# eBay/KPRN

Measured on AMD Instinct MI355X. Metric: paths/sec (train+score) at path_len=6 d=64, higher is better.
Workload: dtype f32

## Files before the change

### kprn_amd/csrc/kprn_api.hip

```cpp
#include <ctype.h>
#include <dlfcn.h>
#include <errno.h>
#include <math.h>
#include <stdio.h>
#include <string.h>

#include <algorithm>
#include <thread>

#include "kprn_internal.h"

static thread_local std::string g_create_error;

ProfScope::ProfScope(kprn_handle* h_, const char* n, hipStream_t on) : h(h_), name(n), strm(on ? on : h_->stream) {
  if (!h->prof_on) return;
  if (!h->prof_filter.empty() && strncmp(n, h->prof_filter.c_str(), h->prof_filter.size()) != 0) return;
  auto get = [&]() {
    hipEvent_t e;
    if (!h->event_pool.empty()) { e = h->event_pool.back(); h->event_pool.pop_back(); }
    else if (hipEventCreate(&e) != hipSuccess) e = nullptr;
    return e;
  };
  a = get(); b = get();
  if (a) hipEventRecord(a, strm);
// ... 1760 lines not shown
    HIP_TRY(hipEventSynchronize(e1));
    float t = 0.f;
    HIP_TRY(hipEventElapsedTime(&t, e0, e1));
    *ms = t / (float)iters;
  } catch (...) { dfree(A); dfree(B); dfree(C); dfree(X); dfree(Z); hipEventDestroy(e0); hipEventDestroy(e1); throw; }
  dfree(A); dfree(B); dfree(C); dfree(X); dfree(Z); hipEventDestroy(e0); hipEventDestroy(e1);
  API_END(h)
}

int kprn_set_option(kprn_handle* h, const char* key, const char* value) {
  API_BEGIN(h)
  KPRN_REQUIRE(key && value, KPRN_E_ARG, "NULL argument");
  if (strcmp(key, "impl") == 0) {
    if (strcmp(value, "auto") == 0) h->impl = 0;
    else if (strcmp(value, "generic") == 0) h->impl = 1;
    else throw KprnError{KPRN_E_ARG, "impl must be auto or generic"};
  } else if (strcmp(key, "prefix_plan") == 0) {
    h->prefix_plan = atoi(value) ? 1 : 0;
  } else if (strcmp(key, "small_tiles") == 0) {
    join_score(h);
    h->small_tiles_on = atoi(value) != 0;
  } else if (strcmp(key, "tile_handover") == 0) {
    const int v = atoi(value);
    KPRN_REQUIRE(v >= 0 && v <= 2, KPRN_E_ARG, "tile_handover must be 0, 1 or 2");
    h->tile_handover = v;
  } else if (strcmp(key, "rank_sort_min") == 0) {
    const int v = atoi(value);
    KPRN_REQUIRE(v >= 257 && v <= 4097, KPRN_E_ARG, "rank_sort_min must be in 257..4097");
    h->rank_sort_min = v;
  } else if (strcmp(key, "adam_merged") == 0) {
    h->adam_merged = atoi(value) != 0;
  } else if (strcmp(key, "bwd_pipe") == 0) {
    h->bwd_pipe = atoi(value) != 0;
  } else if (strcmp(key, "score_dual") == 0) {
    const int v = atoi(value);
    KPRN_REQUIRE(v >= 0 && v <= 2, KPRN_E_ARG, "score_dual must be 0, 1 or 2");
    h->score_dual = v;
  } else if (strcmp(key, "catchup_prefix") == 0) {
    h->catchup_prefix = atoi(value) != 0;
  } else if (strcmp(key, "fused_small_tables") == 0) {
    h->fused_small_tables = atoi(value) != 0;
  } else if (strcmp(key, "persist_layers") == 0) {
    const int v = atoi(value);
    KPRN_REQUIRE(v >= 0 && v <= 2, KPRN_E_ARG, "persist_layers must be 0, 1 or 2");
    h->persist_layers = v;
  } else if (strcmp(key, "small_tables") == 0) {
    h->small_tables = atoi(value) != 0;
  } else if (strcmp(key, "small_tables_fwd") == 0) {
    join_score(h);
    h->small_tables_fwd = atoi(value) != 0;
  } else if (strcmp(key, "head_select") == 0) {
    join_score(h);
    h->head_select = atoi(value) != 0;
  } else if (strcmp(key, "bf16_t_pad") == 0) {
    bf16p::set_t_pad(atoi(value));
  } else if (strcmp(key, "bf16_gemm_regstage") == 0) {
    bf16p::set_gemm_regstage(atoi(value) != 0);
  } else if (strcmp(key, "bf16_gemm_touch") == 0) {
    bf16p::set_gemm_touch(atoi(value));
  } else if (strcmp(key, "bf16_gemm_pingpong") == 0) {
    bf16p::set_gemm_pingpong(atoi(value) != 0);
  } else if (strcmp(key, "bf16_bptt_dxe") == 0) {
    const int v = atoi(value);
    KPRN_REQUIRE(v == 0 || v == 8 || v == 16, KPRN_E_ARG, "bf16_bptt_dxe must be 0, 8 or 16");
    h->bf16_bptt_dxe = v;
  } else if (strcmp(key, "bf16_small_tables") == 0) {
    h->bf16_small_tables = atoi(value) != 0;
  } else if (strcmp(key, "score_rest_before_bptt") == 0) {
    join_score(h);
    h->score_rest_before_bptt = atoi(value) ? 1 : 0;
  } else if (strcmp(key, "score_rest_in_backward") == 0) {
    join_score(h);
    h->score_rest_in_backward = atoi(value) ? 1 : 0;
    h->after_bptt_hook = h->score_rest_in_backward ? score_rest_hook : nullptr;
  } else if (strcmp(key, "score_split") == 0) {
    join_score(h);
    const double f = atof(value);
    KPRN_REQUIRE(f >= 0.0 && f < 1.0, KPRN_E_ARG, "score_split: a fraction in [0, 1)");
    h->score_split = (float)f;
  } else if (strcmp(key, "score_overlap") == 0) {
    join_score(h);
    h->score_overlap = atoi(value) ? 1 : 0;
  } else if (strcmp(key, "loss_accumulate") == 0) {
    h->loss_accumulate = atoi(value) ? 1 : 0;
  } else if (strcmp(key, "inline_upload") == 0) {
    if (strcmp(value, "side") == 0) h->inline_upload_side = 1;
    else if (strcmp(value, "main") == 0) h->inline_upload_side = 0;
    else throw KprnError{KPRN_E_ARG, "inline_upload must be side or main"};
  } else if (strcmp(key, "train_step_return") == 0) {
    if (strcmp(value, "loss") == 0) h->train_step_drain = 0;
    else if (strcmp(value, "drain") == 0) h->train_step_drain = 1;
    else throw KprnError{KPRN_E_ARG, "train_step_return must be loss or drain"};
  } else if (strcmp(key, "feed_build") == 0) {
    if (strcmp(value, "host") == 0) h->feed_build_host = 1;
    else if (strcmp(value, "device") == 0) h->feed_build_host = 0;
    else throw KprnError{KPRN_E_ARG, "feed_build must be host or device"};
  } else if (strcmp(key, "feed_threads") == 0) {
    const int v = atoi(value);
    KPRN_REQUIRE(v >= 1 && v <= 64, KPRN_E_ARG, "feed_threads must be in 1..64");
    h->feed_threads = v;
  } else if (strcmp(key, "feed_workers") == 0) {
    const int v = atoi(value);
    KPRN_REQUIRE(v >= 1 && v <= 64 && !h->feed_pool, KPRN_E_ARG, "feed_workers must be in 1..64 and set before the first feed");
    h->feed_workers = v;
  } else if (strcmp(key, "profile_filter") == 0) {
    h->prof_filter = value;
// ... 40 lines not shown
```

### kprn_amd/csrc/kprn_internal.h

```cpp
#pragma once
#include <stdlib.h>
#include <hip/hip_runtime.h>
#include <stdint.h>
#include <exception>
#include <functional>
#include <future>
#include <string>
#include <vector>
#include <map>

#include "../../include/kprn.h"
#include "philox_dev.h"

#define KPRN_MAX_LAYERS 8

struct KprnError { int code; std::string msg; };
#define HIP_TRY(expr)                                                                     \
  do {                                                                                    \
    hipError_t e__ = (expr);                                                              \
    if (e__ != hipSuccess)                                                                \
      throw KprnError{KPRN_E_DEVICE, std::string(#expr) + ": " + hipGetErrorString(e__)}; \
  } while (0)
#define KPRN_REQUIRE(cond, code, text) \
  do { if (!(cond)) throw KprnError{(code), std::string(text)}; } while (0)
// ... 123 lines not shown
  const int32_t* rows_view = nullptr; const int32_t* count_view = nullptr; const kprn_batch* view_batch = nullptr;
  bool pad_clean = false;
  bool dense_grads_clean = false;
  int64_t caught_serial = -1, caught_step = -1;
  int64_t grads_serial = -1;
  int64_t next_serial = 1;
  int loss_accumulate = 0;
  float* loss_partial = nullptr; int64_t loss_partial_cap = 0; int loss_pending = 0;
  float* loss_mirror = nullptr; int64_t loss_mirror_cap = 0; hipEvent_t ev_loss = nullptr;
  bool loss_early_armed = false; int loss_early_n = 0; int train_step_drain = 0;
  float* probs_mirror = nullptr; int64_t probs_mirror_cap = 0; float* sel_host_armed = nullptr;
  int32_t* dp_mark = nullptr;
  bool dp_fused_update = false, dp_union_pending = false;
  const void* dp_all = nullptr; int dp_world = 0, dp_cap = 0;
  void* dp_comm = nullptr; int dp_rank = 0, dp_nranks = 0;
  int32_t* dp_gather = nullptr; int64_t dp_gather_words = 0;
  bool dp_comm_stream_on = false, dp_begun = false;
  hipStream_t dp_comm_stream = nullptr; hipEvent_t ev_dp_packed = nullptr, ev_dp_gathered = nullptr;
  bool dp_dense_in_pack = false;
  bool dp_saved_dense_in_pack = false, dp_saved_fused_update = false;
  int32_t* pack_buf = nullptr; int64_t pack_cap = 0, pack_words = 0;

  float* d_loss = nullptr;
  float* d_norm2 = nullptr;
  int32_t* d_flag = nullptr;
  float* h_pinned = nullptr;

  Workspace ws;
  float* score_buf = nullptr;
  void* fused_state = nullptr;
  void* bf16_state = nullptr;
  void* bidx_scratch = nullptr; size_t bidx_scratch_bytes = 0;
  hipStream_t feed_stream = nullptr; hipEvent_t ev_feed_fork = nullptr;
  void* feed_scratch = nullptr; size_t feed_scratch_bytes = 0;
  int feed_build_host = 1;
  int feed_workers = 0, feed_threads = 0;
  void* feed_pool = nullptr;
  void* upload_pool = nullptr;
  hipStream_t upload_stream = nullptr;
  int impl = 0;
  int prefix_plan = 1;
  int score_overlap = 0;
  hipStream_t score_stream = nullptr;
  int side_stream_probes = 0;
  hipEvent_t ev_fork = nullptr, ev_score_done = nullptr;
  kprn_batch* dropin_slot[4] = {nullptr, nullptr, nullptr, nullptr};
  int dropin_next_train = 0, dropin_next_score = 0, dropin_last = 0;
  bool dropin_prev_waited = false, dropin_prev_waited_now = false; int inline_upload_side = 1;
  bool inline_side_ok = true;
  bool score_pending = false;
  int bf16_bptt_dxe = 8;
  int persist_layers = 1;
  bool small_tables_fwd = true;
  bool head_select = true;
  bool small_tables = true;
  float* lp_wot = nullptr; int64_t lp_wot_cap = 0;
  float* st_ctmp = nullptr; int64_t st_ctmp_cap = 0;
  bool bf16_small_tables = true;
  bool small_tiles_on = true;
  int tile_handover = 2; int* ho_fault = nullptr;
  bool adam_merged = true;
  bool bwd_pipe = true;
  int score_dual = 2;
  bool catchup_prefix = true;
  bool fused_small_tables = true;
  float score_split = 0.f;
  int score_rest_in_backward = 0;
  int score_rest_before_bptt = 0;
  hipStream_t rest_stream = nullptr; hipEvent_t ev_part1 = nullptr;
  void (*after_bptt_hook)(kprn_handle*) = nullptr;
  const kprn_batch* score_rest_batch = nullptr; int score_rest_cid = 1; int64_t score_rest_tile0 = 0;
  bool last_forward_side = false;
  bool score_on_main = false;
  const kprn_batch* pool_defer_batch = nullptr; int pool_defer_cid = 0;
  float* S2 = nullptr; float* sel2 = nullptr; int64_t cap_N2 = 0, cap_B2 = 0;
  int reserve_cus = 0;
  int32_t last_B = 0;
  float* board = nullptr; int64_t board_n = 0;
  hipEvent_t ev_put = nullptr; bool put_side = false;
  void* rank_buf = nullptr; size_t rank_buf_bytes = 0;
  int rank_sort_min = 512;
  void* rank_pin = nullptr; size_t rank_pin_bytes = 0, rank_pin_off[2] = {0, 0};
  void* explain_buf = nullptr; size_t explain_buf_bytes = 0;
  void* explain_pin = nullptr; size_t explain_pin_bytes = 0;
  std::vector<kprn_graph*> graphs;
  void* pf_buf = nullptr; size_t pf_buf_bytes = 0;
  std::vector<kprn_sampler*> samplers;
  void* ns_buf = nullptr; size_t ns_buf_bytes = 0;

  int deterministic = 0;
  DetScratch det_slab;
  float* det_seg = nullptr; int64_t det_seg_cap = 0;
  float dropout_p = 0.f;
  uint64_t dropout_seed = 0;
  uint32_t drop_draw = 0, drop_draw_cur = 0;
  bool drop_live = false;
  float* det_norm_part = nullptr;

  bool prof_on = false;

  std::string prof_filter;
  std::map<std::string, ProfEntry> prof;
  struct Pending { std::string name; hipEvent_t a, b;  int launches = 1; };
  std::vector<Pending> prof_pending;
  std::vector<hipEvent_t> event_pool;
};
// ... 429 lines not shown
```

### kprn_amd/csrc/lstm_fused_bwd.hip

```cpp
#include <string.h>

#include <memory>

#include "lstm_fused_common.h"

namespace fused {

struct BwdArgs {
  const int32_t* idx; int64_t N; int T, F, nT;
  const float *Wt, *We, *Wr; int dt, de, dr; int Vt, Vr;
  int L, layer;
  const float* WiT;
  const float* WoT;
  const float* save_frag;
  const float* dS;
  const float* wout_row;
  float* gWout_row; float* gbout_c;
  float* DX;
  float* DXe;
  int64_t Npad;
  float* gWi; float* gbi; float* gWo;
  float* gWt; float* gWe; float* gWr;
  float* part;
  unsigned long long* timing;
  int dbg;
  int64_t n_tiles;
  const int32_t* tile_k;
  float* PG;
  HoArgs ho;
  int small_lds;
  float* gG;
  unsigned* pipe_flag;
  int pipe;
};


constexpr int PART = 2 * 256 * 64 + 256;
constexpr int NS_ID = 16;
constexpr int PART_G = PART + 256 * NS_ID;
constexpr int LDD = 4 * DH + 4;
constexpr int DET_PG = 80, DET_SMALL = DET_PG + (KCAP + 1) * PFB, DET_STRIDE = DET_SMALL + 1024;

#ifdef KPRN_TIMING_PROBES
#define KPRN_PROBES_ON 1
#else
#define KPRN_PROBES_ON 0
#endif
#define TPROBE(slot)                                                                 \
  if (KPRN_PROBES_ON && a.timing) {                                                   \
    const unsigned long long now__ = __builtin_amdgcn_s_memtime();                    \
    tacc[slot] += now__ - tlast;                                                      \
    tlast = now__;                                                                    \
  }

struct Pre {
  f32x4 P[6];
  f32x4 up;
  f32x4 bin[4];
  f32x4 bhp[4];
};

__device__ __forceinline__ void gather_load_ident(const BwdArgs& a, const int t, const int32_t* ids, f32x4 (&v)[4]) {
  const int ch = threadIdx.x & 15, c0 = 4 * ch;
  const int32_t* p = ids + t * MT + (threadIdx.x >> 4);
  const float* eb = a.We - a.de + ((ch + 4) & 7) * 4;
#pragma unroll
  for (int k = 0; k < 4; ++k) {
    const f32x4 e = *(const f32x4*)(eb + (int64_t)p[IDS_PLANE<MT> + k * 16] * a.de);
    const int rel = p[2 * IDS_PLANE<MT> + k * 16] - 1, typ = a.Vr + p[k * 16] - 1;
    f32x4 oh;
#pragma unroll
    for (int i = 0; i < 4; ++i) oh[i] = (c0 + i == rel || c0 + i == typ) ? 1.f : 0.f;
    v[k] = (ch < 4) ? oh : ((ch < 12) ? e : f32x4{0.f, 0.f, 0.f, 0.f});
  }
}

template <bool BOTTOM, bool TOP, int NMT, bool IDENT = false, bool DET = false>
__device__ __forceinline__ void bwd_body(const BwdArgs& a, const int bx, const int G_, float* const det_part = nullptr) {
  static_assert(!IDENT || (BOTTOM && !TOP && NMT == 4), "the identity route: bottom layer of two, 64-path tiles");
  constexpr int MTR = 16 * NMT;
  constexpr int NXT = IDENT ? 3 : 4;
  extern __shared__ __attribute__((aligned(16))) float lds[];
  unsigned long long tacc[8] = {0, 0, 0, 0, 0, 0, 0, 0};
  unsigned long long tlast = (KPRN_PROBES_ON && a.timing) ? __builtin_amdgcn_s_memtime() : 0ull;
  float* dA_t = lds;
  float* in_t = dA_t + MT * LDD;
  int32_t* ids = (int32_t*)(in_t + (BOTTOM ? MT * LDA : 0));
  constexpr int IDS_BUF = MT * MAXT_LDS * 4;
  float* pg = (float*)(ids + (BOTTOM ? 2 * IDS_BUF : 0));

  const int tid = threadIdx.x;
  const int lane = tid & 63;
  const int j = __builtin_amdgcn_readfirstlane(tid >> 6);
  const int arow = lane & 15, ag = lane >> 4;
  const int T = a.T, L = a.L, ly = a.layer;
  const HoPlan ho = ho_plan(a.ho, a.tile_k, a.n_tiles, T, 1, bx, G_);
  auto mof = [&](const int i) -> int { return IDENT ? ((i + 2 * (j >> 1)) & 3) : i; };
  if (IDENT && bx == 0) for (int c = tid; c < 256 * NS_ID; c += 256) a.gG[c] = 0.f;

  f32x4 wiT[16], woT[16];
  {
    const float* wi_row = a.WiT + (int64_t)((IDENT ? a.dt + 16 * (j & 1) : j * 16) + arow) * (4 * DH) + ag * 4;
    const float* wo_row = a.WoT + (int64_t)(j * 16 + arow) * (4 * DH) + ag * 4;
#pragma unroll
    for (int S = 0; S < 16; ++S) { wiT[S] = *(const f32x4*)(wi_row + S * 16); woT[S] = *(const f32x4*)(wo_row + S * 16); }
#pragma unroll
    for (int S = 0; S < 16; ++S) { asm volatile("" : "+a"(wiT[S])); asm volatile("" : "+a"(woT[S])); }
  }
  f32x4 dwi[4][4], dwo[4][4];
  float dbias[4];
#pragma unroll
  for (int q = 0; q < 4; ++q) {
    dbias[q] = 0.f;
#pragma unroll
    for (int nt = 0; nt < 4; ++nt) {
      dwi[q][nt] = f32x4{0.f, 0.f, 0.f, 0.f}; dwo[q][nt] = f32x4{0.f, 0.f, 0.f, 0.f};
      if (nt < NXT) asm volatile("" : "+a"(dwi[q][nt]));
      asm volatile("" : "+a"(dwo[q][nt]));
    }
  }

  const int64_t frag_unit = (int64_t)NPL * 256;
  const int64_t frag_mt_stride = (int64_t)T * L * 4 * frag_unit;
  const int wcls = (j * 16 < a.dt) ? 0 : ((j * 16 < a.dt + a.de) ? 1 : 2);
  GatherSrc gsrc;
  if (BOTTOM) gsrc = gather_src(a);
  const float wout_c = TOP ? a.wout_row[j * 16 + arow] : 0.f;
  float gwo = 0.f, gbo = 0.f;
  for (int c = tid; c < (KCAP + 1) * PFB; c += 256) pg[c] = 0.f;
  f32x4 sacc[2] = {f32x4{0.f, 0.f, 0.f, 0.f}, f32x4{0.f, 0.f, 0.f, 0.f}};
  TPROBE(0)

  const int64_t n_mine = (a.n_tiles > (int64_t)bx) ? (a.n_tiles - 1 - bx) / G_ + 1 : 0;
  float* const ho_slot = a.ho.state + (int64_t)ho.slot * HO_STATE + threadIdx.x * 4;
  auto own_of = [&](const int64_t it) -> int64_t {
    const int64_t ti = TOP ? n_mine - 1 - it : ((ho.role == 1) ? (it + 1 < n_mine ? it + 1 : 0) : it);
    return (int64_t)bx + ti * G_;
  };
  int ipar = 1;
  int k0_req = 0;
  auto request_tile = [&](const int64_t tl, const int buf) {
    if (a.tile_k) k0_req = a.tile_k[tl];
    if (BOTTOM) ids_stage_dma<256, MTR>(a.idx, a.N, T, a.F, a.nT, tl, ids + buf * IDS_BUF);
  };
  if (n_mine > 0) request_tile(ho.role == 2 ? ho.tile : own_of(0), 0);
  for (int64_t it = 0; it < n_mine; ++it) {
    const int64_t own_tile = own_of(it);
    const bool late = ho.role == 1 && own_tile == (int64_t)bx;
    const bool early = ho.role == 2 && it == 0;
    int64_t tile, n0;
    int k0, Te;
    const float* frag_tile;
    float* dx_tile;
    auto retarget = [&](const int64_t tl) {
      tile = tl;
      n0 = tl * MTR;
      k0 = a.tile_k ? __builtin_amdgcn_readfirstlane(k0_req) : 0;
      Te = T - k0;
      frag_tile = a.save_frag + tl * NMT * frag_mt_stride + (int64_t)k0 * L * 4 * frag_unit + lane * 4;
      dx_tile = a.DX + (((tl * NMT) * T + k0) * 4 + j) * 256 + lane * 4;
    };
    retarget(early ? ho.tile : own_tile);
    auto frag_ptr = [&](int mt, int t, int l, int w, int plane) -> const float* {
      return frag_tile + mt * frag_mt_stride + ((int64_t)(t * L + l) * 4 + w) * frag_unit + plane * 256;
    };
    f32x4 P[6], up, bin[4], bhp[4];
    auto load_P = [&](const int slot, int t) {
      const int mt = mof(slot);
#pragma unroll
      for (int k = 0; k < 6; ++k) P[k] = *(const f32x4*)frag_ptr(mt, t, ly, j, k);
      if constexpr (!TOP && NMT == 1) {
        if (a.pipe == 2) {
          const unsigned* fl = a.pipe_flag + tile * MAXT_LDS + (k0 + t);
          const long long t0 = wall_clock64();
          while (__hip_atomic_load(fl, __ATOMIC_RELAXED, __HIP_MEMORY_SCOPE_AGENT) != a.ho.epoch) {
            __builtin_amdgcn_s_sleep(4);
            if (wall_clock64() - t0 > HO_TIMEOUT_TICKS) {
              if (threadIdx.x == 0) __hip_atomic_store(a.ho.fault, 1, __ATOMIC_RELAXED, __HIP_MEMORY_SCOPE_SYSTEM);
              break;
            }
          }
          asm volatile("" ::: "memory");
          up = ho_load4(dx_tile + (mt * T + t) * 1024);
        } else up = *(const f32x4*)(dx_tile + (mt * T + t) * 1024);
      } else if (!TOP) up = *(const f32x4*)(dx_tile + (mt * T + t) * 1024);
    };
    auto load_B = [&](int nt, const int slot, int t, bool has_hp) {
      const int mt = mof(slot);
      if (!BOTTOM) bin[nt] = *(const f32x4*)frag_ptr(mt, t, ly - 1, nt, 6);
      if (has_hp) bhp[nt] = *(const f32x4*)frag_ptr(mt, t - 1, ly, nt, 6);
    };
    auto load_bin_lds = [&](int nt, const int slot) {
      if (nt >= NXT) return;
      const int mt = mof(slot);
#pragma unroll
      for (int r = 0; r < 4; ++r) bin[nt][r] = in_t[(mt * 16 + ag * 4 + r) * LDA + nt * 16 + arow];
    };
    auto gather_load_x = [&](const int t, f32x4 (&v)[MTR * 16 / 256]) {
      if constexpr (IDENT) gather_load_ident(a, t, ids + ipar * IDS_BUF, v);
      else gather_load_planes<256, MTR>(a, gsrc, tile, t, ids + ipar * IDS_BUF, v);
    };
    const int tt_hi = late ? Te - 1 - ho.d : Te - 1;
    f32x4 dc[NMT], dh[NMT];
    auto init_state = [&]() {
#pragma unroll
      for (int m = 0; m < NMT; ++m) {
        dc[m] = f32x4{0.f, 0.f, 0.f, 0.f};
        dh[m] = f32x4{0.f, 0.f, 0.f, 0.f};
        if (TOP) {
          const f32x4 hf = *(const f32x4*)(frag_tile + m * frag_mt_stride + ((int64_t)((Te - 1) * L + ly) * 4 + j) * frag_unit + 6 * 256);
#pragma unroll
          for (int r = 0; r < 4; ++r) {
            const int64_t n = n0 + m * 16 + ag * 4 + r;
            const float d = (n < a.N) ? a.dS[n] : 0.f;
            dh[m][r] = d * wout_c;
            gwo += d * hf[r];
            gbo += d;
          }
        }
      }
    };
    if (__builtin_expect(late, 0)) {
      ho_wait(a.ho, ho.slot);
#pragma unroll
      for (int m = 0; m < NMT; ++m) { dh[m] = ho_load4(ho_slot + m * 1024); dc[m] = ho_load4(ho_slot + (NMT + m) * 1024); }
    } else {
      init_state();
    }
    auto tile_prologue = [&](const int tt_first, const int64_t next) {
      ipar ^= 1;
      if (BOTTOM) {
        asm volatile("s_waitcnt vmcnt(0)" ::: "memory");
        lds_barrier();
        f32x4 nin[MTR * 16 / 256];
        gather_load_x(k0 + tt_first, nin);
        gather_store<256, MTR>(in_t, nin);
      }
      if (next >= 0) request_tile(next, ipar ^ 1);
      if (BOTTOM) lds_barrier();
    };
    tile_prologue(tt_hi, early ? own_tile : (it + 1 < n_mine ? own_of(it + 1) : (int64_t)-1));
    TPROBE(1)
    load_P(0, tt_hi);
#pragma unroll
    for (int nt = 0; nt < 4; ++nt) load_B(nt, 0, tt_hi, tt_hi > 0);

    auto step = [&](auto rec_tag, const int t) {
      constexpr bool REC = decltype(rec_tag)::value;
      if (BOTTOM) {
#pragma unroll
        for (int nt = 0; nt < 4; ++nt) load_bin_lds(nt, 0);
      }
#pragma unroll
      for (int mt = 0; mt < NMT; ++mt) {
        f32x4 dhv = dh[mt];
        if (!TOP) dhv += up;
        const f32x4 dC = dc[mt] + dhv * P[4];
        f32x4 dA[4];
        dA[0] = dC * P[0];
        dA[1] = dC * P[1];
        dA[2] = dC * P[2];
        dA[3] = dhv * P[3];
        dc[mt] = dC * P[5];
#pragma unroll
        for (int q = 0; q < 4; ++q) {
#pragma unroll
          for (int r = 0; r < 4; ++r) dA_t[(mof(mt) * 16 + ag * 4 + r) * LDD + q * DH + j * 16 + arow] = dA[q][r];
          dbias[q] += (dA[q][0] + dA[q][1]) + (dA[q][2] + dA[q][3]);
        }
        __builtin_amdgcn_sched_barrier(0);
        TPROBE(7)
        if (mt < NMT - 1) load_P(mt + 1, t);
        else if (REC) load_P(0, t - 1);
#pragma unroll
        for (int nt = 0; nt < 4; ++nt) {
#pragma unroll
          for (int r = 0; r < 4; ++r)
#pragma unroll
            for (int q = 0; q < 4; ++q) {
              if (nt < NXT) KPRN_MFMA_ACC_A(dwi[q][nt], dA[q][r], bin[nt][r]);
              if (REC) KPRN_MFMA_ACC_A(dwo[q][nt], dA[q][r], bhp[nt][r]);
            }
          __builtin_amdgcn_sched_barrier(0);
          if (mt < NMT - 1) { load_B(nt, mt + 1, t, REC); if (BOTTOM) load_bin_lds(nt, mt + 1); }
          else if (REC) load_B(nt, 0, t - 1, t > 1);
        }
        TPROBE(2)
      }
      lds_barrier();
      if (!REC && k0 > 0) {
        float cs0 = 0.f, cs1 = 0.f;
#pragma unroll 8
        for (int row = 0; row < MTR; row += 2) { cs0 += dA_t[row * LDD + tid]; cs1 += dA_t[(row + 1) * LDD + tid]; }
        pg[k0 * PFB + tid] += cs0 + cs1;
      }
      TPROBE(3)
      f32x4 nin[MTR * 16 / 256];
      if (BOTTOM && REC) gather_load_x(k0 + t - 1, nin);

      f32x4 ax[4], ah[4];
      if constexpr (NMT < 4) {
#pragma unroll
        for (int q = NMT; q < 4; ++q) { ax[q] = f32x4{0.f, 0.f, 0.f, 0.f}; ah[q] = f32x4{0.f, 0.f, 0.f, 0.f}; }
      }
      if constexpr (IDENT) { ax[2] = f32x4{0.f, 0.f, 0.f, 0.f}; ax[3] = f32x4{0.f, 0.f, 0.f, 0.f}; }
      if constexpr (IDENT) {
        const float* abase = dA_t + arow * LDD + ag * 4;
        auto afrag = [&](const int slot, const int S) { return *(const f32x4*)(abase + mof(slot) * 16 * LDD + S * 16); };
        if (REC) {
          f32x4 p0 = afrag(0, 0), p1, p2, p3;
#pragma unroll
          for (int S = 0; S < 16; ++S) {
#pragma unroll
            for (int i = 0; i < 2; ++i) {
              const f32x4 a4 = (i == 0) ? p0 : p1;
              if (S == 0) { KPRN_MFMA_Z(ax[i], a4[0], wiT[S][0]); KPRN_MFMA_Z(ah[i], a4[0], woT[S][0]); }
              else { KPRN_MFMA(ax[i], a4[0], wiT[S][0]); KPRN_MFMA(ah[i], a4[0], woT[S][0]); }
              KPRN_MFMA(ax[i], a4[1], wiT[S][1]); KPRN_MFMA(ah[i], a4[1], woT[S][1]);
              if (i == 0) p1 = afrag(1, S);
              else { p2 = afrag(2, S); p3 = afrag(3, S); }
              KPRN_MFMA(ax[i], a4[2], wiT[S][2]); KPRN_MFMA(ah[i], a4[2], woT[S][2]);
              KPRN_MFMA(ax[i], a4[3], wiT[S][3]); KPRN_MFMA(ah[i], a4[3], woT[S][3]);
            }
            const f32x4 a2 = p2, a3 = p3;
            if (S == 0) { KPRN_MFMA_Z(ah[2], a2[0], woT[S][0]); KPRN_MFMA_Z(ah[3], a3[0], woT[S][0]); }
            else { KPRN_MFMA(ah[2], a2[0], woT[S][0]); KPRN_MFMA(ah[3], a3[0], woT[S][0]); }
            KPRN_MFMA(ah[2], a2[1], woT[S][1]); KPRN_MFMA(ah[3], a3[1], woT[S][1]);
            if (S + 1 < 16) p0 = afrag(0, S + 1);
            KPRN_MFMA(ah[2], a2[2], woT[S][2]); KPRN_MFMA(ah[3], a3[2], woT[S][2]);
            KPRN_MFMA(ah[2], a2[3], woT[S][3]); KPRN_MFMA(ah[3], a3[3], woT[S][3]);
          }
        } else {
          f32x4 p0 = afrag(0, 0), p1 = afrag(1, 0);
#pragma unroll
          for (int S = 0; S < 16; ++S) {
            const f32x4 a0 = p0, a1 = p1;
            if (S == 0) { KPRN_MFMA_Z(ax[0], a0[0], wiT[S][0]); KPRN_MFMA_Z(ax[1], a1[0], wiT[S][0]); }
            else { KPRN_MFMA(ax[0], a0[0], wiT[S][0]); KPRN_MFMA(ax[1], a1[0], wiT[S][0]); }
// ... 6 lines not shown
      } else {
        const float* abase = dA_t + arow * LDD + ag * 4;
        if (REC) {
          f32x4 apre = *(const f32x4*)(abase);
#pragma unroll
          for (int S = 0; S < 16; ++S) {
#pragma unroll
            for (int mt = 0; mt < NMT; ++mt) {
              const f32x4 a4 = apre;
              const int gn = S * NMT + mt + 1;
              if (S == 0) { KPRN_MFMA_Z(ax[mt], a4[0], wiT[S][0]); KPRN_MFMA_Z(ah[mt], a4[0], woT[S][0]); }
              else { KPRN_MFMA(ax[mt], a4[0], wiT[S][0]); KPRN_MFMA(ah[mt], a4[0], woT[S][0]); }
              KPRN_MFMA(ax[mt], a4[1], wiT[S][1]); KPRN_MFMA(ah[mt], a4[1], woT[S][1]);
              if (gn < 16 * NMT) apre = *(const f32x4*)(abase + (gn % NMT) * 16 * LDD + (gn / NMT) * 16);
              KPRN_MFMA(ax[mt], a4[2], wiT[S][2]); KPRN_MFMA(ah[mt], a4[2], woT[S][2]);
              KPRN_MFMA(ax[mt], a4[3], wiT[S][3]); KPRN_MFMA(ah[mt], a4[3], woT[S][3]);
            }
          }
        } else if constexpr (NMT == 1) {
          f32x4 ap0 = *(const f32x4*)(abase), ap1 = *(const f32x4*)(abase + 16);
#pragma unroll
          for (int S = 0; S < 16; S += 2) {
            const f32x4 a0 = ap0, a1 = ap1;
            if (S == 0) { KPRN_MFMA_Z(ax[0], a0[0], wiT[S][0]); KPRN_MFMA_Z(ax[1], a1[0], wiT[S + 1][0]); }
            else { KPRN_MFMA(ax[0], a0[0], wiT[S][0]); KPRN_MFMA(ax[1], a1[0], wiT[S + 1][0]); }
            KPRN_MFMA(ax[0], a0[1], wiT[S][1]); KPRN_MFMA(ax[1], a1[1], wiT[S + 1][1]);
            if (S + 2 < 16) { ap0 = *(const f32x4*)(abase + (S + 2) * 16); ap1 = *(const f32x4*)(abase + (S + 3) * 16); }
            KPRN_MFMA(ax[0], a0[2], wiT[S][2]); KPRN_MFMA(ax[1], a1[2], wiT[S + 1][2]);
            KPRN_MFMA(ax[0], a0[3], wiT[S][3]); KPRN_MFMA(ax[1], a1[3], wiT[S + 1][3]);
          }
        } else {
          f32x4 ap0 = *(const f32x4*)(abase), ap1 = *(const f32x4*)(abase + 16 * LDD);
#pragma unroll
          for (int S = 0; S < 16; ++S) {
#pragma unroll
            for (int mp = 0; mp < 2; ++mp) {
              const f32x4 a0 = ap0, a1 = ap1;
              const int gn = S * 2 + mp + 1;
              if (S == 0) { KPRN_MFMA_Z(ax[2 * mp], a0[0], wiT[S][0]); KPRN_MFMA_Z(ax[2 * mp + 1], a1[0], wiT[S][0]); }
              else { KPRN_MFMA(ax[2 * mp], a0[0], wiT[S][0]); KPRN_MFMA(ax[2 * mp + 1], a1[0], wiT[S][0]); }
              KPRN_MFMA(ax[2 * mp], a0[1], wiT[S][1]); KPRN_MFMA(ax[2 * mp + 1], a1[1], wiT[S][1]);
              if (gn < 32) {
                ap0 = *(const f32x4*)(abase + ((gn & 1) * 2) * 16 * LDD + (gn >> 1) * 16);
                ap1 = *(const f32x4*)(abase + ((gn & 1) * 2 + 1) * 16 * LDD + (gn >> 1) * 16);
              }
              KPRN_MFMA(ax[2 * mp], a0[2], wiT[S][2]); KPRN_MFMA(ax[2 * mp + 1], a1[2], wiT[S][2]);
              KPRN_MFMA(ax[2 * mp], a0[3], wiT[S][3]); KPRN_MFMA(ax[2 * mp + 1], a1[3], wiT[S][3]);
            }
          }
        }
      }
      KPRN_MFMA_DRAIN();
      KPRN_PIN_V4(ax);
      if (REC) KPRN_PIN_V4(ah);
      if constexpr (NMT == 1) { if (!REC) ax[0] += ax[1]; }
      if (BOTTOM && REC) gather_store<256, MTR>(in_t, nin);
      const bool compact = !IDENT && BOTTOM && a.DXe != nullptr && wcls == 1;
#pragma unroll
      for (int mt = 0; mt < NMT; ++mt) {
        if (REC) dh[mt] = ah[mt];
        if constexpr (IDENT) continue;
        if constexpr (TOP && !BOTTOM && NMT == 1) {
          if (a.pipe == 1) ho_store4(dx_tile + (mt * T + t) * 1024, ax[mt]);
          else *(f32x4*)(dx_tile + (mt * T + t) * 1024) = ax[mt];
        } else
        if (!compact && !(BOTTOM && a.small_lds && wcls != 1)) *(f32x4*)(dx_tile + (mt * T + t) * 1024) = ax[mt];
      }
      if (compact) {
        float* de_row = a.DXe + ((n0 + ag * 4) * T + k0 + t) * (int64_t)a.de + (j * 16 + arow - a.dt);
#pragma unroll
        for (int mt = 0; mt < NMT; ++mt)
#pragma unroll
          for (int r = 0; r < 4; ++r) de_row[(int64_t)(mt * 16 + r) * T * a.de] = ax[mt][r];
      }
      if constexpr (IDENT) {
        float* de_row = a.DXe + ((n0 + ag * 4) * T + k0 + t) * (int64_t)a.de + 16 * (j & 1) + arow;
#pragma unroll
        for (int i = 0; i < 2; ++i)
#pragma unroll
          for (int r = 0; r < 4; ++r) de_row[(int64_t)(mof(i) * 16 + r) * T * a.de] = ax[i][r];
      }
      if (!IDENT && BOTTOM && a.small_lds && wcls != 1) {
        const int32_t* idp = ids + ipar * IDS_BUF + ((wcls == 0) ? 0 : 2) * IDS_PLANE<MTR> + (k0 + t) * MTR + ag * 4;
#pragma unroll
        for (int mt = 0; mt < NMT; ++mt) {
          const int4 id4 = *(const int4*)(idp + mt * 16);
          const float o0 = (id4.x - 1 == arow) ? 1.f : 0.f, o1 = (id4.y - 1 == arow) ? 1.f : 0.f;
          const float o2 = (id4.z - 1 == arow) ? 1.f : 0.f, o3 = (id4.w - 1 == arow) ? 1.f : 0.f;
          KPRN_MFMA_VV(sacc[0], o0, ax[mt][0]);
          KPRN_MFMA_VV(sacc[1], o1, ax[mt][1]);
          KPRN_MFMA_VV(sacc[0], o2, ax[mt][2]);
          KPRN_MFMA_VV(sacc[1], o3, ax[mt][3]);
        }
        KPRN_MFMA_DRAIN();
        asm volatile("" : "+v"(sacc[0]), "+v"(sacc[1]));
      }
      TPROBE(4)
      if constexpr (TOP && !BOTTOM && NMT == 1) {
        if (a.pipe == 1) asm volatile("s_waitcnt vmcnt(0)" ::: "memory");
      }
      lds_barrier();
      if constexpr (TOP && !BOTTOM && NMT == 1) {
        if (a.pipe == 1 && tid == 0) __hip_atomic_store(a.pipe_flag + tile * MAXT_LDS + (k0 + t), a.ho.epoch, __ATOMIC_RELAXED, __HIP_MEMORY_SCOPE_AGENT);
      }
      TPROBE(5)
    };
    int tt_sw = early ? Te - ho.d : -1;
    int tt_pub = -1;
    for (int tt = tt_hi; tt > 0; --tt) {
      step(std::true_type{}, tt);
      if (__builtin_expect(tt == tt_pub, 0)) { ho_publish(a.ho, ho.slot); tt_pub = -1; }
      if (__builtin_expect(tt == tt_sw, 0)) {
#pragma unroll
        for (int m = 0; m < NMT; ++m) { ho_store4(ho_slot + m * 1024, dh[m]); ho_store4(ho_slot + (NMT + m) * 1024, dc[m]); }
        retarget(own_tile);
        init_state();
        tile_prologue(Te - 1, n_mine > 1 ? own_of(1) : (int64_t)-1);
        load_P(0, Te - 1);
#pragma unroll
        for (int nt = 0; nt < 4; ++nt) load_B(nt, 0, Te - 1, Te > 1);
        tt = Te;
        tt_sw = -1;
        tt_pub = Te - 1;
      }
    }
    step(std::false_type{}, 0);
    if (k0 > 0) {
      float cs = 0.f;
#pragma unroll
      for (int m = 0; m < NMT; ++m) cs += (dc[m][0] + dc[m][1]) + (dc[m][2] + dc[m][3]);
      cs += __shfl_xor(cs, 16, 64);
      cs += __shfl_xor(cs, 32, 64);
      if (ag == 0) pg[k0 * PFB + 4 * DH + j * 16 + arow] += cs;
    }
  }
  float* const det_slab = DET ? det_part + (int64_t)bx * DET_STRIDE : nullptr;
  if (a.tile_k) {
    lds_barrier();
    for (int c = PFB + tid; c < (KCAP + 1) * PFB; c += 256) {
      const float v = pg[c];
      if constexpr (DET) det_slab[DET_PG + c] = v;
      else if (v != 0.f) unsafeAtomicAdd(a.PG + c, v);
    }
  }
  if (!IDENT && BOTTOM && a.small_lds && wcls != 1) {
    const f32x4 sg = sacc[0] + sacc[1];
    const int V = (wcls == 0) ? a.Vt : a.Vr, width = (wcls == 0) ? a.dt : a.dr;
    float* g = (DET ? det_slab + DET_SMALL + ((wcls == 0) ? 0 : a.Vt * a.dt) : ((wcls == 0) ? a.gWt : a.gWr)) + (j * 16 + arow - ((wcls == 0) ? 0 : a.dt + a.de));
#pragma unroll
    for (int i = 0; i < 4; ++i) {
      const int v = 4 * ag + i;
      if constexpr (DET) { if (v < V) g[(int64_t)v * width] = sg[i]; }
      else if (v < V && sg[i] != 0.f) unsafeAtomicAdd(g + (int64_t)v * width, sg[i]);
    }
  }

  KPRN_MFMA_DRAIN();
#pragma unroll
  for (int q = 0; q < 4; ++q) {
    if constexpr (IDENT) asm volatile("" : "+a"(dwi[q][0]), "+a"(dwi[q][1]), "+a"(dwi[q][2]), "+a"(dwo[q][0]), "+a"(dwo[q][1]), "+a"(dwo[q][2]), "+a"(dwo[q][3]));
    else KPRN_PIN_A8(dwi[q], dwo[q]);
  }
  {
    float* pw = a.part + (int64_t)bx * PART_G;
#pragma unroll
    for (int q = 0; q < 4; ++q) {
#pragma unroll
      for (int nt = 0; nt < 4; ++nt) {
#pragma unroll
        for (int r = 0; r < 4; ++r) {
          const int64_t grow = (int64_t)q * DH + j * 16 + ag * 4 + r;
          if constexpr (IDENT) {
            if (nt == 0) pw[PART + grow * NS_ID + arow] = dwi[q][0][r];
            else if (nt < NXT) pw[grow * DH + a.dt + (nt - 1) * 16 + arow] = dwi[q][nt][r];
            else {
              pw[grow * DH + (arow < a.dt ? arow : arow + a.de)] = 0.f;
              pw[grow * DH + (16 + arow < a.dt ? 16 + arow : 16 + arow + a.de)] = 0.f;
            }
          } else {
            pw[grow * DH + nt * 16 + arow] = dwi[q][nt][r];
          }
          pw[256 * 64 + grow * DH + nt * 16 + arow] = dwo[q][nt][r];
        }
      }
      float v = dbias[q];
      v += __shfl_xor(v, 16, 64);
      v += __shfl_xor(v, 32, 64);
      if (ag == 0) pw[2 * 256 * 64 + q * DH + j * 16 + arow] = v;
    }
  }
  if (TOP) {
    float v = gwo;
    v += __shfl_xor(v, 16, 64);
    v += __shfl_xor(v, 32, 64);
    if constexpr (DET) { if (ag == 0) det_slab[j * 16 + arow] = v; }
    else if (ag == 0) unsafeAtomicAdd(a.gWout_row + j * 16 + arow, v);
    float bsum = gbo;
    bsum += __shfl_xor(bsum, 16, 64);
    bsum += __shfl_xor(bsum, 32, 64);
    if constexpr (DET) { if (j == 0 && lane == 0) det_slab[DH] = bsum; }
    else if (j == 0 && lane == 0) unsafeAtomicAdd(a.gbout_c, bsum);
  }
  TPROBE(6)
  if (KPRN_PROBES_ON && a.timing && tid == 0) {
    for (int k = 0; k < 8; ++k) a.timing[(int64_t)bx * 8 + k] = tacc[k];
  }
}

template <bool BOTTOM, bool TOP, int NMT>
__global__ __launch_bounds__(256, 1) void k_lstm_bwd(BwdArgs a) { bwd_body<BOTTOM, TOP, NMT>(a, (int)blockIdx.x, (int)gridDim.x); }
__global__ __launch_bounds__(256, 1) void k_lstm_bwd_ident(BwdArgs a) { bwd_body<true, false, 4, true>(a, (int)blockIdx.x, (int)gridDim.x); }

template <int NMT>
__global__ __launch_bounds__(256, 1) void k_lstm_bwd_dual(BwdArgs top, BwdArgs bottom, int g) {
  if ((int)blockIdx.x < g) bwd_body<false, true, NMT>(top, (int)blockIdx.x, g);
  else bwd_body<true, false, NMT>(bottom, (int)blockIdx.x - g, g);
}

template <bool BOTTOM, bool TOP, int NMT, bool IDENT>
__global__ __launch_bounds__(256, 1) void k_lstm_bwd_det(BwdArgs a, float* det_part) {
  bwd_body<BOTTOM, TOP, NMT, IDENT, true>(a, (int)blockIdx.x, (int)gridDim.x, det_part);
}
template <int NMT>
__global__ __launch_bounds__(256, 1) void k_lstm_bwd_dual_det(BwdArgs top, BwdArgs bottom, int g, float* det_top, float* det_bottom) {
  if ((int)blockIdx.x < g) bwd_body<false, true, NMT, false, true>(top, (int)blockIdx.x, g, det_top);
  else bwd_body<true, false, NMT, false, true>(bottom, (int)blockIdx.x - g, g, det_bottom);
}
struct DetJoin { int nseg, nslab; float* dst[6]; const float* src[6]; int n[6]; int blk0[7]; };
__global__ __launch_bounds__(256) void k_det_join(DetJoin a) {
  constexpr int DEPTH = 16;
  int sgm = 0;
  while (sgm + 1 < a.nseg && (int)blockIdx.x >= a.blk0[sgm + 1]) ++sgm;
  const int i = ((int)blockIdx.x - a.blk0[sgm]) * 256 + threadIdx.x;
  if (i >= a.n[sgm]) return;
  const float* __restrict__ src = a.src[sgm] + i;
  float acc = 0.f;
  for (int w0 = 0; w0 < a.nslab; w0 += DEPTH) {
    float x[DEPTH];
#pragma unroll
    for (int u = 0; u < DEPTH; ++u) x[u] = src[(int64_t)(w0 + u < a.nslab ? w0 + u : a.nslab - 1) * DET_STRIDE];
#pragma unroll
    for (int u = 0; u < DEPTH; ++u) if (w0 + u < a.nslab) acc += x[u];
  }
  a.dst[sgm][i] += acc;
}

struct ScatArgs {
  const int32_t* idx; int64_t N; int T, F, nT;
  int dt, de, dr, Vt, Vr;
  const float* DX;
  float *gWt, *gWe, *gWr;
  const int32_t* tile_k;
  int do_small, do_entity;
  float* part_small;
  int64_t n_tiles;
};

__global__ __launch_bounds__(256) void k_embed_scatter_frag(ScatArgs a) {
  extern __shared__ __attribute__((aligned(16))) float lds[];
  float* dxt = lds;
  int32_t* ids = (int32_t*)(dxt + MT * LDA);
  float* small_g = (float*)(ids + MT * 4);
  const int tid = threadIdx.x, lane = tid & 63, w0 = tid >> 6;
  const int arow = lane & 15, ag = lane >> 4;
  const int T = a.T, D = a.dt + a.de + a.dr;
  const int n_small = a.Vt * a.dt + a.Vr * a.dr;
  const bool small_in_lds = a.part_small != nullptr && a.do_small;
  if (small_in_lds) for (int i = tid; i < n_small; i += 256) small_g[i] = 0.f;
  const int e0 = a.dt, e1 = a.dt + a.de;
  const int col = tid & 63, rg = tid >> 6;
  const int64_t n_items = a.n_tiles * T;
  for (int64_t item = blockIdx.x; item < n_items; item += gridDim.x) {
    const int64_t tile = item / T;
    const int t = (int)(item - tile * T);
// ... 70 lines not shown
    __syncthreads();
    for (int i = tid; i < n_small; i += 256) a.part_small[(int64_t)blockIdx.x * n_small + i] = small_g[i];
  }
}

__global__ __launch_bounds__(256) void k_reduce_small(const float* __restrict__ part, int nslab, int n_small, int nt_small, float* __restrict__ gWt, float* __restrict__ gWr) {
  __shared__ float red[16][17];
  const int e = threadIdx.x & 15, sl = threadIdx.x >> 4;
  const int i = blockIdx.x * 16 + e;
  float acc = 0.f;
  if (i < n_small) for (int s = sl; s < nslab; s += 16) acc += part[(int64_t)s * n_small + i];
  red[sl][e] = acc;
  __syncthreads();
  if (sl == 0 && i < n_small) {
    float v = 0.f;
#pragma unroll
    for (int k = 0; k < 16; ++k) v += red[k][e];
    if (i < nt_small) unsafeAtomicAdd(gWt + i, v); else unsafeAtomicAdd(gWr + (i - nt_small), v);
  }
}

__global__ void k_reduce_partials(bidx::SlabReduce a) { bidx::slab_reduce_block(a, blockIdx.x, blockIdx.y, blockIdx.z); }

struct TransArgs { const float* W[4]; float* WT[4]; };
__global__ void k_transpose_256x64(TransArgs a) {
  const int i = blockIdx.x * blockDim.x + threadIdx.x;
  if (i >= 64 * 256) return;
  const int n = i >> 8, k = i & 255;
  a.WT[blockIdx.y][i] = a.W[blockIdx.y][k * 64 + n];
}

bool transpose_job(kprn_handle* h, kk::TransposeJob* tj) {
  State* s = st(h);
  if (!s->wt_dirty) return false;
  const int L = h->cfg.L;
  if (!s->WT) HIP_TRY(kprn_dev_malloc((void**)&s->WT, (size_t)2 * 2 * 64 * 256 * sizeof(float)));
  tj->n = 2 * L;
  for (int m = 0; m < 4; ++m) {
    const int l = (m >> 1) < L ? (m >> 1) : 0;
    tj->W[m] = h->dense + ((m & 1) ? h->layer[l].Wo : h->layer[l].Wi);
    tj->WT[m] = s->WT + (size_t)(l * 2 + (m & 1)) * 64 * 256;
  }
  s->wt_dirty = false;
  return true;
}

bool bwd_supported(const kprn_handle* h, int T) { return fwd_supported(h, T); }

template <bool BOTTOM, bool TOP, int NMT = 4, bool IDENT = false>
static void launch_bwd(kprn_handle* h, const BwdArgs& a, int grid, float* det_part = nullptr) {
  size_t lds_bytes = (size_t)MT * LDD * sizeof(float);
  if (BOTTOM) lds_bytes += (size_t)MT * LDA * sizeof(float) + 2 * (MT * MAXT_LDS * 4) * sizeof(int32_t);
  lds_bytes += (size_t)(KCAP + 1) * PFB * sizeof(float);
  if (det_part) {
    if constexpr (BOTTOM || TOP) {
      static PerDeviceOnce det_attr_done;
      if (det_attr_done.need())
        HIP_TRY(hipFuncSetAttribute((const void*)k_lstm_bwd_det<BOTTOM, TOP, NMT, IDENT>, hipFuncAttributeMaxDynamicSharedMemorySize, (int)lds_bytes));
      hipLaunchKernelGGL((k_lstm_bwd_det<BOTTOM, TOP, NMT, IDENT>), dim3(grid), dim3(256), lds_bytes, h->stream, a, det_part);
      HIP_TRY(hipGetLastError());
      return;
    }
    throw KprnError{KPRN_E_UNSUPPORTED, "deterministic: the fused path has no middle layer"};
  }
  static PerDeviceOnce attr_done;
  const void* fn = IDENT ? (const void*)k_lstm_bwd_ident : (const void*)k_lstm_bwd<BOTTOM, TOP, NMT>;
  if (attr_done.need()) HIP_TRY(hipFuncSetAttribute(fn, hipFuncAttributeMaxDynamicSharedMemorySize, (int)lds_bytes));
  if constexpr (IDENT) hipLaunchKernelGGL(k_lstm_bwd_ident, dim3(grid), dim3(256), lds_bytes, h->stream, a);
  else hipLaunchKernelGGL((k_lstm_bwd<BOTTOM, TOP, NMT>), dim3(grid), dim3(256), lds_bytes, h->stream, a);
  HIP_TRY(hipGetLastError());
}

void backward(kprn_handle* h, const kprn_batch* b, int cid) {
  const kprn_config& c = h->cfg;
  State* s = st(h);
  const int64_t N = b->N;
  const int T = b->T, L = c.L;
  hipStream_t strm = h->stream;
  if (N > s->cap_Nb || T > s->cap_Tb) {
    HIP_TRY(hipStreamSynchronize(strm));
    if (s->DX) hipFree(s->DX);
    const int64_t cn = std::max<int64_t>(N, s->cap_Nb);
    const int ct = std::max(T, s->cap_Tb);
    HIP_TRY(kprn_dev_malloc((void**)&s->DX, (size_t)ct * (cn + 2 * MT) * DH * sizeof(float)));
    if (s->DXe) hipFree(s->DXe);
    HIP_TRY(kprn_dev_malloc((void**)&s->DXe, (size_t)(ct * (cn + 2 * MT) + KCAP) * c.de * sizeof(float)));
    s->cap_Nb = cn; s->cap_Tb = ct;
  }
  if (!s->part) HIP_TRY(kprn_dev_malloc((void**)&s->part, (size_t)2 * s->num_cu * PART_G * sizeof(float)));
  const bool det = h->deterministic;
  if (det && !s->det_part) HIP_TRY(kprn_dev_malloc((void**)&s->det_part, (size_t)2 * s->num_cu * DET_STRIDE * sizeof(float)));
  static const bool want_timing = KPRN_DEV_ENV("KPRN_TIMING") != nullptr;
  if (want_timing && !s->timing) HIP_TRY(kprn_dev_malloc((void**)&s->timing, (size_t)s->num_cu * 12 * sizeof(unsigned long long)));
  if (s->wt_dirty) {
    ProfScope ps(h, "weight_transpose");
    kk::TransposeJob tj;
    transpose_job(h, &tj);
    TransArgs ta;
    for (int m = 0; m < 4; ++m) { ta.W[m] = tj.W[m < tj.n ? m : 0]; ta.WT[m] = tj.WT[m < tj.n ? m : 0]; }
    hipLaunchKernelGGL(k_transpose_256x64, dim3(64, tj.n), dim3(256), 0, strm, ta);
    HIP_TRY(hipGetLastError());
  }
  float* gd = h->g_dense;
  const bool small = small_tiles(h, N, b->tile_k != nullptr);
  const int64_t n_tiles64 = (N + MT - 1) / MT;
  const int64_t n_tiles = small ? (N + 15) / 16 : n_tiles64;
// ... 207 lines not shown
```

Measured before the change: 51.25 million.

## Stage backward h fragments through LDS with async global-to-LDS loads

Adds a default-on path for the fused LSTM backward kernel (64-path tiles, top or bottom layer of two). It prefetches the previous-step hidden and lower-layer input fragments into a double-buffered LDS area using global_load_lds_dwordx4, so the register loads of B operands inside the MFMA loop become LDS reads. The aim is to hide global-load latency on the recurrent critical path and free VGPRs. In exchange it uses extra LDS, adds vmcnt waits and barriers, and relies on inline asm that manipulates m0.

Measured after the change: 51.27 million, median of 5. No clear change (+0.0%).

```diff
diff --git a/kprn_amd/csrc/kprn_api.hip b/kprn_amd/csrc/kprn_api.hip
--- a/kprn_amd/csrc/kprn_api.hip
+++ b/kprn_amd/csrc/kprn_api.hip
@@ -1836,6 +1836,8 @@
   } else if (strcmp(key, "head_select") == 0) {
     join_score(h);
     h->head_select = atoi(value) != 0;
+  } else if (strcmp(key, "bwd_h_lds") == 0) {
+    h->bwd_h_lds = atoi(value) != 0;
   } else if (strcmp(key, "bf16_t_pad") == 0) {
     bf16p::set_t_pad(atoi(value));
   } else if (strcmp(key, "bf16_gemm_regstage") == 0) {
diff --git a/kprn_amd/csrc/kprn_internal.h b/kprn_amd/csrc/kprn_internal.h
--- a/kprn_amd/csrc/kprn_internal.h
+++ b/kprn_amd/csrc/kprn_internal.h
@@ -199,6 +199,7 @@
   int bf16_bptt_dxe = 8;
   int persist_layers = 1;
   bool small_tables_fwd = true;
+  bool bwd_h_lds = true;
   bool head_select = true;
   bool small_tables = true;
   float* lp_wot = nullptr; int64_t lp_wot_cap = 0;
diff --git a/kprn_amd/csrc/lstm_fused_bwd.hip b/kprn_amd/csrc/lstm_fused_bwd.hip
--- a/kprn_amd/csrc/lstm_fused_bwd.hip
+++ b/kprn_amd/csrc/lstm_fused_bwd.hip
@@ -75,9 +75,12 @@
   }
 }
 
-template <bool BOTTOM, bool TOP, int NMT, bool IDENT = false, bool DET = false>
+template <bool TOP> constexpr int HB_FLOATS = 4 * (TOP ? 2 : 1) * 4 * 256;
+template <bool BOTTOM, bool TOP, int NMT, bool IDENT = false, bool DET = false, bool HLDS = false>
 __device__ __forceinline__ void bwd_body(const BwdArgs& a, const int bx, const int G_, float* const det_part = nullptr) {
   static_assert(!IDENT || (BOTTOM && !TOP && NMT == 4), "the identity route: bottom layer of two, 64-path tiles");
+  static_assert(!HLDS || (NMT == 4 && BOTTOM != TOP), "h fragments through LDS: 64-path tiles, top or bottom layer of two");
+  constexpr int HB_SRC = TOP ? 2 : 1, HB = HB_FLOATS<TOP>;
   constexpr int MTR = 16 * NMT;
   constexpr int NXT = IDENT ? 3 : 4;
   extern __shared__ __attribute__((aligned(16))) float lds[];
@@ -88,6 +91,7 @@
   int32_t* ids = (int32_t*)(in_t + (BOTTOM ? MT * LDA : 0));
   constexpr int IDS_BUF = MT * MAXT_LDS * 4;
   float* pg = (float*)(ids + (BOTTOM ? 2 * IDS_BUF : 0));
+  float* hb = pg + (KCAP + 1) * PFB;
 
   const int tid = threadIdx.x;
   const int lane = tid & 63;
@@ -185,10 +189,32 @@
         } else up = *(const f32x4*)(dx_tile + (mt * T + t) * 1024);
       } else if (!TOP) up = *(const f32x4*)(dx_tile + (mt * T + t) * 1024);
     };
-    auto load_B = [&](int nt, const int slot, int t, bool has_hp) {
+    auto load_B = [&](int nt, const int slot, int t, bool has_hp, const bool tile_start = false) {
+#ifdef KPRN_EXP_BOWN
+      if (NMT == 4 && !tile_start && (KPRN_EXP_BOWN == 2 ? nt != 0 : nt != j)) return;
+#endif
       const int mt = mof(slot);
       if (!BOTTOM) bin[nt] = *(const f32x4*)frag_ptr(mt, t, ly - 1, nt, 6);
       if (has_hp) bhp[nt] = *(const f32x4*)frag_ptr(mt, t - 1, ly, nt, 6);
+    };
+    const unsigned hb_base = lds_offset_of(hb);
+    auto hb_request = [&](const int p, const int t) {
+      const int mt = TOP ? (p >> 1) : p;
+      const bool hp = TOP ? (p & 1) != 0 : true;
+      if (hp && t == 0) return;
+      const float* src = hp ? frag_ptr(mt, t - 1, ly, j, 6) : frag_ptr(mt, t, ly - 1, j, 6);
+      const unsigned dst = (unsigned)__builtin_amdgcn_readfirstlane((int)(hb_base + (unsigned)((t & 1) * HB + ((mt * HB_SRC + (TOP && hp ? 1 : 0)) * 4 + j) * 256) * 4u));
+      unsigned keep;
+      asm volatile("s_mov_b32 %0, m0\n\ts_mov_b32 m0, %2\n\ts_nop 0\n\tglobal_load_lds_dwordx4 %1, off\n\ts_mov_b32 m0, %0" : "=&s"(keep) : "v"(src), "s"(dst) : "memory");
+    };
+    auto hb_fill = [&](const int t) {
+#pragma unroll
+      for (int p = 0; p < 4 * HB_SRC; ++p) hb_request(p, t);
+    };
+    auto load_B_hb = [&](int nt, const int slot, int t, bool has_hp) {
+      const float* b = hb + (t & 1) * HB + ((mof(slot) * HB_SRC) * 4 + nt) * 256 + lane * 4;
+      if (TOP) bin[nt] = *(const f32x4*)b;
+      if (has_hp) bhp[nt] = *(const f32x4*)(b + (TOP ? 4 * 256 : 0));
     };
     auto load_bin_lds = [&](int nt, const int slot) {
       if (nt >= NXT) return;
@@ -229,6 +255,8 @@
     }
     auto tile_prologue = [&](const int tt_first, const int64_t next) {
       ipar ^= 1;
+      if (HLDS) hb_fill(tt_first);
+      if (HLDS && !BOTTOM) { asm volatile("s_waitcnt vmcnt(0)" ::: "memory"); lds_barrier(); }
       if (BOTTOM) {
         asm volatile("s_waitcnt vmcnt(0)" ::: "memory");
         lds_barrier();
@@ -243,13 +271,17 @@
     TPROBE(1)
     load_P(0, tt_hi);
 #pragma unroll
-    for (int nt = 0; nt < 4; ++nt) load_B(nt, 0, tt_hi, tt_hi > 0);
+    for (int nt = 0; nt < 4; ++nt) if (!HLDS) load_B(nt, 0, tt_hi, tt_hi > 0, true);
 
     auto step = [&](auto rec_tag, const int t) {
       constexpr bool REC = decltype(rec_tag)::value;
       if (BOTTOM) {
 #pragma unroll
         for (int nt = 0; nt < 4; ++nt) load_bin_lds(nt, 0);
+      }
+      if constexpr (HLDS) {
+#pragma unroll
+        for (int nt = 0; nt < 4; ++nt) load_B_hb(nt, 0, t, REC);
       }
 #pragma unroll
       for (int mt = 0; mt < NMT; ++mt) {
@@ -282,8 +314,13 @@
               if (REC) KPRN_MFMA_ACC_A(dwo[q][nt], dA[q][r], bhp[nt][r]);
             }
           __builtin_amdgcn_sched_barrier(0);
-          if (mt < NMT - 1) { load_B(nt, mt + 1, t, REC); if (BOTTOM) load_bin_lds(nt, mt + 1); }
-          else if (REC) load_B(nt, 0, t - 1, t > 1);
+          if constexpr (HLDS) {
+            if (mt < NMT - 1) { load_B_hb(nt, mt + 1, t, REC); if (BOTTOM) load_bin_lds(nt, mt + 1); }
+            if (REC && nt < HB_SRC) hb_request(mt * HB_SRC + nt, t - 1);
+          } else {
+            if (mt < NMT - 1) { load_B(nt, mt + 1, t, REC); if (BOTTOM) load_bin_lds(nt, mt + 1); }
+            else if (REC) load_B(nt, 0, t - 1, t > 1);
+          }
         }
         TPROBE(2)
       }
@@ -396,6 +433,7 @@
       }
       KPRN_MFMA_DRAIN();
       KPRN_PIN_V4(ax);
+      if (HLDS && REC) asm volatile("s_waitcnt vmcnt(0)" ::: "memory");
       if (REC) KPRN_PIN_V4(ah);
       if constexpr (NMT == 1) { if (!REC) ax[0] += ax[1]; }
       if (BOTTOM && REC) gather_store<256, MTR>(in_t, nin);
@@ -462,7 +500,7 @@
         tile_prologue(Te - 1, n_mine > 1 ? own_of(1) : (int64_t)-1);
         load_P(0, Te - 1);
 #pragma unroll
-        for (int nt = 0; nt < 4; ++nt) load_B(nt, 0, Te - 1, Te > 1);
+        for (int nt = 0; nt < 4; ++nt) if (!HLDS) load_B(nt, 0, Te - 1, Te > 1, true);
         tt = Te;
         tt_sw = -1;
         tt_pub = Te - 1;
@@ -561,9 +599,16 @@
   else bwd_body<true, false, NMT>(bottom, (int)blockIdx.x - g, g);
 }
 
+template <bool BOTTOM, bool TOP, bool IDENT>
+__global__ __launch_bounds__(256, 1) void k_lstm_bwd_hlds(BwdArgs a) { bwd_body<BOTTOM, TOP, 4, IDENT, false, true>(a, (int)blockIdx.x, (int)gridDim.x); }
+
 template <bool BOTTOM, bool TOP, int NMT, bool IDENT>
 __global__ __launch_bounds__(256, 1) void k_lstm_bwd_det(BwdArgs a, float* det_part) {
   bwd_body<BOTTOM, TOP, NMT, IDENT, true>(a, (int)blockIdx.x, (int)gridDim.x, det_part);
+}
+template <bool BOTTOM, bool TOP, bool IDENT>
+__global__ __launch_bounds__(256, 1) void k_lstm_bwd_hlds_det(BwdArgs a, float* det_part) {
+  bwd_body<BOTTOM, TOP, 4, IDENT, true, true>(a, (int)blockIdx.x, (int)gridDim.x, det_part);
 }
 template <int NMT>
 __global__ __launch_bounds__(256, 1) void k_lstm_bwd_dual_det(BwdArgs top, BwdArgs bottom, int g, float* det_top, float* det_bottom) {
@@ -740,6 +785,20 @@
   size_t lds_bytes = (size_t)MT * LDD * sizeof(float);
   if (BOTTOM) lds_bytes += (size_t)MT * LDA * sizeof(float) + 2 * (MT * MAXT_LDS * 4) * sizeof(int32_t);
   lds_bytes += (size_t)(KCAP + 1) * PFB * sizeof(float);
+  if constexpr (NMT == 4 && BOTTOM != TOP) {
+    if (h->bwd_h_lds) {
+      constexpr size_t base = (size_t)MT * LDD * 4 + (BOTTOM ? (size_t)MT * LDA * 4 + 2 * (MT * MAXT_LDS * 4) * 4 : 0) + (size_t)(KCAP + 1) * PFB * 4;
+      static_assert(base + 2 * HB_FLOATS<TOP> * 4 <= 160 * 1024, "one workgroup per CU: 160 KiB of LDS");
+      lds_bytes += 2 * HB_FLOATS<TOP> * sizeof(float);
+      static PerDeviceOnce hlds_attr_done[2];
+      const void* fn = det_part ? (const void*)k_lstm_bwd_hlds_det<BOTTOM, TOP, IDENT> : (const void*)k_lstm_bwd_hlds<BOTTOM, TOP, IDENT>;
+      if (hlds_attr_done[det_part ? 1 : 0].need()) HIP_TRY(hipFuncSetAttribute(fn, hipFuncAttributeMaxDynamicSharedMemorySize, (int)lds_bytes));
+      if (det_part) hipLaunchKernelGGL((k_lstm_bwd_hlds_det<BOTTOM, TOP, IDENT>), dim3(grid), dim3(256), lds_bytes, h->stream, a, det_part);
+      else hipLaunchKernelGGL((k_lstm_bwd_hlds<BOTTOM, TOP, IDENT>), dim3(grid), dim3(256), lds_bytes, h->stream, a);
+      HIP_TRY(hipGetLastError());
+      return;
+    }
+  }
   if (det_part) {
     if constexpr (BOTTOM || TOP) {
       static PerDeviceOnce det_attr_done;
```
